# georgesterpu/avsr-tf1

Hardware: AMD Instinct MI355X
Metric: utterances/sec (train step) at B=64 T_a=500 T_v=75 (higher is better)
Workload: dtype f32; 1 GPU; c4: AV dual-attention (bimodal) video 1x256 + audio 3x256 uni-LSTM, scaled_luong, B=64 T_a=500x80 T_v=75 L=40; utterances_per_gpu=64, global_batch=64, T_a=500, F_a=80, T_v=75, F_v=128, T_dec=40, parallelism=dp1, video_frontend=resnet_cnn, launch=hipgraph, dropout=True

## Files before the change

### avsr-tf1_amd/csrc/gemm.hip

```cpp
#include "common.h"
#include "avsr_hip.h"
#include "prof.h"

namespace avsr {

constexpr int BM = 128, BN = 128, BK = 16;

struct MatView {
  const float* p;
  long ld;
  int T;
  long ldo;
  __device__ __forceinline__ const float* row(int r) const {
    return T ? p + (long)(r / T) * ldo + (long)(r % T) * ld : p + (long)r * ld;
  }
};

struct GemmArgs {
  MatView A, B;
  float* C; long ldc; int Tc; long ldoc;
  const float* bias;
  const float* alpha_dev;
  int M, N, K;
  int ta, tb;
  float alpha, beta;
  int splitk, kper;
  float* ws;
  long sA, sB, sC;
  int batch;
  float* cs_out; float cs_beta; float* cs_ws;
};

#define G_OOB ((int)0x80000000)
template <bool KC, bool VEC>
struct OperandLoader {
  __amdgpu_buffer_rsrc_t rs;
  int off[2];
  int q[2], r[2];
  bool ok;
  int ldb, ldob, T;
  int tail;
  int MN, mn;

  __device__ __forceinline__ void init(const MatView& S, int mn0, int k0, int MN_) {
    const int tid = threadIdx.x;
    rs = __builtin_amdgcn_make_buffer_rsrc(const_cast<float*>(S.p), 0, 0x80000000u, 0x00020000);
    ldb = (int)S.ld * 4; ldob = (int)S.ldo * 4; T = S.T; MN = MN_;
    if (KC) {
      mn = mn0 + (tid & 127);
      ok = mn < MN;
      const int ro = T ? (mn / T) * ldob + (mn % T) * ldb : mn * ldb;
#pragma unroll
      for (int p = 0; p < 2; ++p) off[p] = ro + (k0 + 4 * ((tid >> 7) + 2 * p)) * 4;
    } else {
      mn = mn0 + 4 * (tid & 31);
      ok = mn < MN;
#pragma unroll
      for (int p = 0; p < 2; ++p) {
        const int k = k0 + (tid >> 5) + 8 * p;
        q[p] = T ? k / T : 0; r[p] = T ? k % T : k;
        off[p] = mn * 4;
      }
    }
  }
  __device__ __forceinline__ void load(int k0, int kend, f32x4 (&out)[2]) {
    const int tid = threadIdx.x;
#pragma unroll
    for (int p = 0; p < 2; ++p) {
      int o, k;
      if (KC) { k = k0 + 4 * ((tid >> 7) + 2 * p); o = off[p]; off[p] += BK * 4; }
      else {
        k = k0 + (tid >> 5) + 8 * p;
        o = (T ? q[p] * ldob + r[p] * ldb : r[p] * ldb) + off[p];
        r[p] += BK;
        if (T) { while (r[p] >= T) { r[p] -= T; ++q[p]; } }
      }
      const bool in = ok && k < kend;
      typedef unsigned int u32x4_ __attribute__((ext_vector_type(4)));
      if (VEC) {
        out[p] = __builtin_bit_cast(f32x4, (u32x4_)__builtin_amdgcn_raw_buffer_load_b128(rs, in ? o : G_OOB, 0, 0));
      } else {
#pragma unroll
        for (int e = 0; e < 4; ++e) {
          const bool ine = in && (KC ? k + e < kend : mn + e < MN);
          out[p][e] = __builtin_bit_cast(float, (unsigned)__builtin_amdgcn_raw_buffer_load_b32(rs, ine ? o + 4 * e : G_OOB, 0, 0));
        }
      }
    }
  }
};

template <bool KC>
__device__ __forceinline__ void store_tile(float* T, const f32x4 (&r)[2]) {
  const int tid = threadIdx.x;
#pragma unroll
  for (int p = 0; p < 2; ++p) {
    if (KC) {
      const int mn = tid & 127;
      const int k = 4 * ((tid >> 7) + 2 * p);
#pragma unroll
      for (int e = 0; e < 4; ++e) T[(k + e) * BM + mn] = r[p][e];
    } else {
      const int k = (tid >> 5) + 8 * p;
      const int mn = 4 * (tid & 31);
      st4(&T[k * BM + mn], r[p]);
    }
  }
}

template <bool AKC, bool BKC, bool VECA, bool VECB>
__device__ __forceinline__ void gemm_body(const GemmArgs& g, const int bx, const int by, const int z) {
  __shared__ __attribute__((aligned(16))) float lds[2][2][BK * BM];
  const int tid = threadIdx.x, lane = tid & 63, wave = tid >> 6;
  const int wm = wave >> 1, wn = wave & 1;
  const int bz = z / g.splitk, sz = z % g.splitk;
  MatView A = g.A, B = g.B;
  A.p += (long)bz * g.sA;
  B.p += (long)bz * g.sB;
  const int m0 = by * BM, n0 = bx * BN;
  const int kbeg = sz * g.kper;
  const int kend = min(g.K, kbeg + g.kper);

  f32x16 acc[2][2];
#pragma unroll
  for (int i = 0; i < 2; ++i)
#pragma unroll
    for (int j = 0; j < 2; ++j)
#pragma unroll
      for (int r = 0; r < 16; ++r) acc[i][j][r] = 0.f;

  f32x4 ra[2][2], rb[2][2];
  OperandLoader<AKC, VECA> la;
  OperandLoader<BKC, VECB> lb;
  la.init(A, m0, kbeg, g.M);
  lb.init(B, n0, kbeg, g.N);
  la.load(kbeg, kend, ra[0]);
  lb.load(kbeg, kend, rb[0]);
  la.load(kbeg + BK, kend, ra[1]);
  lb.load(kbeg + BK, kend, rb[1]);
  const bool do_cs = !BKC && g.cs_out != nullptr && by == 0;
  f32x4 csum = {0.f, 0.f, 0.f, 0.f};
  store_tile<AKC>(lds[0][0], ra[0]);
  store_tile<BKC>(lds[0][1], rb[0]);
  if (do_cs) csum += rb[0][0] + rb[0][1];
  __syncthreads();

  auto ktile = [&](int k0, int buf, f32x4 (&ra_next)[2], f32x4 (&rb_next)[2], f32x4 (&ra_free)[2], f32x4 (&rb_free)[2]) {
    la.load(k0 + 2 * BK, kend, ra_free);
    lb.load(k0 + 2 * BK, kend, rb_free);
    const float* As = lds[buf][0];
    const float* Bs = lds[buf][1];
#pragma unroll
    for (int kk = 0; kk < BK / 2; ++kk) {
      const int k = 2 * kk + (lane >> 5);
      const float a0 = As[k * BM + wm * 64 + (lane & 31)];
      const float a1 = As[k * BM + wm * 64 + 32 + (lane & 31)];
      const float b0 = Bs[k * BN + wn * 64 + (lane & 31)];
      const float b1 = Bs[k * BN + wn * 64 + 32 + (lane & 31)];
      acc[0][0] = __builtin_amdgcn_mfma_f32_32x32x2f32(a0, b0, acc[0][0], 0, 0, 0);
      acc[0][1] = __builtin_amdgcn_mfma_f32_32x32x2f32(a0, b1, acc[0][1], 0, 0, 0);
      acc[1][0] = __builtin_amdgcn_mfma_f32_32x32x2f32(a1, b0, acc[1][0], 0, 0, 0);
      acc[1][1] = __builtin_amdgcn_mfma_f32_32x32x2f32(a1, b1, acc[1][1], 0, 0, 0);
    }
    store_tile<AKC>(lds[buf ^ 1][0], ra_next);
    store_tile<BKC>(lds[buf ^ 1][1], rb_next);
    if (do_cs) csum += rb_next[0] + rb_next[1];
    asm volatile("s_waitcnt lgkmcnt(0)\n\ts_barrier" ::: "memory");
  };
  for (int k0 = kbeg; k0 < kend; k0 += 2 * BK) {
    ktile(k0, 0, ra[1], rb[1], ra[0], rb[0]);
    if (k0 + BK < kend) ktile(k0 + BK, 1, ra[0], rb[0], ra[1], rb[1]);
  }

  if (!BKC && g.cs_out != nullptr) {
    float* red = &lds[0][0][0];
    if (do_cs) st4(red + (tid >> 5) * BN + 4 * (tid & 31), csum);
    __syncthreads();
    if (do_cs && tid < BN) {
      float v = 0.f;
#pragma unroll
      for (int r = 0; r < 8; ++r) v += red[r * BN + tid];
      const int col = n0 + tid;
      if (col < g.N) {
        if (g.splitk > 1) g.cs_ws[(long)z * g.N + col] = v;
        else g.cs_out[col] = g.cs_beta != 0.f ? v + g.cs_beta * g.cs_out[col] : v;
      }
    }
    __syncthreads();
  }
  const bool split = g.splitk > 1;
  const float alpha = g.alpha_dev ? g.alpha * g.alpha_dev[0] : g.alpha;
  const unsigned mTc = (g.Tc > 1 && g.M < 65536) ? (unsigned)(((1ull << 32) / (unsigned)g.Tc) + 1ull) : 0u;
  if (split) {
#pragma unroll
    for (int i = 0; i < 2; ++i)
#pragma unroll
      for (int j = 0; j < 2; ++j) {
        const int col = n0 + wn * 64 + j * 32 + (lane & 31);
        if (col >= g.N) continue;
        const int rbase = m0 + wm * 64 + i * 32 + 4 * (lane >> 5);
#pragma unroll
        for (int r = 0; r < 16; ++r) {
          const int row = rbase + (r & 3) + 8 * (r >> 2);
          if (row < g.M) g.ws[((long)z * g.M + row) * g.N + col] = acc[i][j][r];
        }
      }
    return;
  }
  const __amdgpu_buffer_rsrc_t c_rs = __builtin_amdgcn_make_buffer_rsrc(g.C + (long)bz * g.sC, 0, 0x80000000u, 0x00020000);
  int co[2][8];
  float old[2][8];
  auto prep = [&](int t, int (&cot)[8], float (&oldt)[8]) {
    const int i = t >> 2, j = (t >> 1) & 1, h = t & 1;
    const int col = n0 + wn * 64 + j * 32 + (lane & 31);
    const int rbase = m0 + wm * 64 + i * 32 + 4 * (lane >> 5);
#pragma unroll
    for (int rr = 0; rr < 8; ++rr) {
      const int r = h * 8 + rr;
      const int row = rbase + (r & 3) + 8 * (r >> 2);
      int o;
      if (!g.Tc) o = row * (int)g.ldc;
      else {
        const int qd = mTc ? (int)__umulhi((unsigned)row, mTc) : (g.Tc == 1 ? row : row / g.Tc);
        o = qd * (int)g.ldoc + (row - qd * g.Tc) * (int)g.ldc;
      }
      cot[rr] = (row < g.M && col < g.N) ? (o + col) * 4 : G_OOB;
    }
    if (g.beta != 0.f) {
#pragma unroll
      for (int rr = 0; rr < 8; ++rr) oldt[rr] = __builtin_bit_cast(float, (unsigned)__builtin_amdgcn_raw_buffer_load_b32(c_rs, cot[rr], 0, 0));
    }
  };
  prep(0, co[0], old[0]);
#pragma unroll
  for (int t = 0; t < 8; ++t) {
    if (t + 1 < 8) prep(t + 1, co[(t + 1) & 1], old[(t + 1) & 1]);
    const int i = t >> 2, j = (t >> 1) & 1, h = t & 1;
    const int col = n0 + wn * 64 + j * 32 + (lane & 31);
    const float bias_v = (g.bias && col < g.N) ? g.bias[col] : 0.f;
#pragma unroll
    for (int rr = 0; rr < 8; ++rr) {
      float v = alpha * acc[i][j][h * 8 + rr];
      if (g.beta != 0.f) v += g.beta * old[t & 1][rr];
      v += bias_v;
      __builtin_amdgcn_raw_buffer_store_b32(__builtin_bit_cast(unsigned, v), c_rs, co[t & 1][rr], 0, 0);
    }
  }
}

template <bool AKC, bool BKC, bool VECA, bool VECB>
__global__ __launch_bounds__(256, 3) void gemm_f32_kernel(GemmArgs g) {
  gemm_body<AKC, BKC, VECA, VECB>(g, blockIdx.x, blockIdx.y, blockIdx.z);
}

#define GEMM_GROUP_MAX 8
struct GemmGroup { int n; int blk_off[GEMM_GROUP_MAX + 1]; int gx[GEMM_GROUP_MAX], gy[GEMM_GROUP_MAX]; int red_off[GEMM_GROUP_MAX + 1]; GemmArgs g[GEMM_GROUP_MAX]; };

template <bool AKC, bool BKC, bool VECA, bool VECB>
__global__ __launch_bounds__(256, 3) void gemm_f32_group_kernel(const GemmGroup G) {
  int p = 0;
#pragma unroll
  for (int k = 1; k < GEMM_GROUP_MAX; ++k) if (k < G.n && (int)blockIdx.x >= G.blk_off[k]) p = k;
  p = __builtin_amdgcn_readfirstlane(p);
  const int b = blockIdx.x - G.blk_off[p];
  const int gx = G.gx[p], gy = G.gy[p];
  const int bx = b % gx, by = (b / gx) % gy, z = b / (gx * gy);
  gemm_body<AKC, BKC, VECA, VECB>(G.g[p], bx, by, z);
}

__device__ __forceinline__ void splitk_reduce_body(const GemmArgs& g, const long first, const long stride) {
  const long total = (long)g.batch * g.M * g.N;
  if (g.cs_out) {
    for (long col = first; col < g.N; col += stride) {
      float v = 0.f;
      int zz = 0;
      for (; zz + 8 <= g.splitk; zz += 8) {
        float w[8];
#pragma unroll
        for (int u = 0; u < 8; ++u) w[u] = g.cs_ws[(long)(zz + u) * g.N + col];
#pragma unroll
        for (int u = 0; u < 8; ++u) v += w[u];
      }
      for (; zz < g.splitk; ++zz) v += g.cs_ws[(long)zz * g.N + col];
      g.cs_out[col] = g.cs_beta != 0.f ? v + g.cs_beta * g.cs_out[col] : v;
    }
  }
  const bool vec = (g.N & 3) == 0 && ((uintptr_t)g.ws & 15) == 0 && ((uintptr_t)g.C & 15) == 0 && (g.ldc & 3) == 0 && (g.sC & 3) == 0 &&
                   (g.Tc == 0 || (g.ldoc & 3) == 0) && (!g.bias || ((uintptr_t)g.bias & 15) == 0);
  if (vec) {
    const long zs = (long)g.M * g.N;
    const float al = g.alpha_dev ? g.alpha * g.alpha_dev[0] : g.alpha;
    for (long i = first * 4; i < total; i += stride * 4) {
      const int col = (int)(i % g.N);
      const int row = (int)((i / g.N) % g.M);
      const int bz = (int)(i / zs);
      const float* w = g.ws + ((long)bz * g.splitk * g.M + row) * g.N + col;
      f32x4 s = {0.f, 0.f, 0.f, 0.f};
      int z = 0;
      for (; z + 8 <= g.splitk; z += 8) {
        f32x4 a[8];
#pragma unroll
        for (int u = 0; u < 8; ++u) a[u] = ld4(w + (z + u) * zs);
#pragma unroll
        for (int u = 0; u < 8; ++u) s += a[u];
      }
      for (; z < g.splitk; ++z) s += ld4(w + z * zs);
      float* c = g.C + (long)bz * g.sC +
                 (g.Tc ? (long)(row / g.Tc) * g.ldoc + (long)(row % g.Tc) * g.ldc : (long)row * g.ldc) + col;
      f32x4 v = al * s;
      if (g.beta != 0.f) v += g.beta * ld4(c);
      if (g.bias) v += ld4(g.bias + col);
      st4(c, v);
    }
    return;
  }
  for (long i = first; i < total; i += stride) {
    const int col = (int)(i % g.N);
    const int row = (int)((i / g.N) % g.M);
    const int bz = (int)(i / ((long)g.M * g.N));
    const float* w = g.ws + ((long)bz * g.splitk * g.M + row) * g.N + col;
    const long zs = (long)g.M * g.N;
    float s = 0.f;
    int z = 0;
    for (; z + 4 <= g.splitk; z += 4) {
      const float a0 = w[z * zs], a1 = w[(z + 1) * zs], a2 = w[(z + 2) * zs], a3 = w[(z + 3) * zs];
      s = (((s + a0) + a1) + a2) + a3;
    }
    for (; z < g.splitk; ++z) s += w[z * zs];
    float* c = g.C + (long)bz * g.sC +
               (g.Tc ? (long)(row / g.Tc) * g.ldoc + (long)(row % g.Tc) * g.ldc : (long)row * g.ldc) + col;
    float v = (g.alpha_dev ? g.alpha * g.alpha_dev[0] : g.alpha) * s;
    if (g.beta != 0.f) v += g.beta * *c;
    if (g.bias) v += g.bias[col];
    *c = v;
  }
}
__global__ void gemm_splitk_reduce_kernel(GemmArgs g) {
  splitk_reduce_body(g, (long)blockIdx.x * blockDim.x + threadIdx.x, (long)gridDim.x * blockDim.x);
}
__global__ void gemm_splitk_reduce_group_kernel(const GemmGroup G) {
  int p = 0;
#pragma unroll
  for (int k = 1; k < GEMM_GROUP_MAX; ++k) if (k < G.n && (int)blockIdx.x >= G.red_off[k]) p = k;
  p = __builtin_amdgcn_readfirstlane(p);
  if (G.g[p].splitk <= 1) return;
  const int nb = G.red_off[p + 1] - G.red_off[p];
  splitk_reduce_body(G.g[p], (long)(blockIdx.x - G.red_off[p]) * blockDim.x + threadIdx.x, (long)nb * blockDim.x);
}

static bool vec_ok(const avsr_mat* m, bool contig_is_k, int MN, int K) {
  const int contig = contig_is_k ? K : MN;
  return (((uintptr_t)m->ptr) % 16 == 0) && (m->ld % 4 == 0) && (contig % 4 == 0) && (m->T == 0 || m->ldo % 4 == 0);
}

}

static int gemm_prepare(const avsr_gemm_desc* d, avsr::GemmArgs& g, dim3* grid, int* cls) {
  using namespace avsr;
  if (!d || d->M <= 0 || d->N <= 0 || d->K < 0 || !d->A.ptr || !d->B.ptr || !d->C.ptr) return AVSR_ERR_ARG;
  g.A = MatView{d->A.ptr, d->A.ld, d->A.T, d->A.ldo};
  g.B = MatView{d->B.ptr, d->B.ld, d->B.T, d->B.ldo};
  g.C = d->C.ptr; g.ldc = d->C.ld; g.Tc = d->C.T; g.ldoc = d->C.ldo;
  g.bias = d->bias;
  g.alpha_dev = d->alpha_dev;
  g.M = d->M; g.N = d->N; g.K = d->K;
  g.ta = d->trans_a; g.tb = d->trans_b;
  g.alpha = d->alpha; g.beta = d->beta;
  g.batch = d->batch > 0 ? d->batch : 1;
  g.sA = d->stride_a; g.sB = d->stride_b; g.sC = d->stride_c;
  int splitk = d->splitk > 0 ? d->splitk : 1;
  if (splitk > 1 && (!d->workspace || d->workspace_floats < (long)g.batch * splitk * g.M * g.N)) return AVSR_ERR_ARG;
  int kper = ((g.K + splitk - 1) / splitk + BK - 1) / BK * BK;
  if (kper <= 0) kper = BK;
  splitk = (g.K + kper - 1) / kper;
  if (splitk < 1) splitk = 1;
  g.splitk = splitk; g.kper = kper; g.ws = d->workspace;
  g.cs_out = d->colsum; g.cs_beta = d->colsum_beta; g.cs_ws = nullptr;
  if (g.cs_out) {
    if (g.tb || g.batch != 1) return AVSR_ERR_UNSUPPORTED;
    if (splitk > 1) {
      if (d->workspace_floats < (long)splitk * g.M * g.N + (long)splitk * g.N) return AVSR_ERR_ARG;
      g.cs_ws = d->workspace + (long)splitk * g.M * g.N;
    }
  }
  const bool va = vec_ok(&d->A, g.ta == 0, g.M, g.K);
  const bool vb = vec_ok(&d->B, g.tb != 0, g.N, g.K);
  *grid = dim3((g.N + BN - 1) / BN, (g.M + BM - 1) / BM, g.batch * splitk);
  if ((long)d->A.ld * 4 >= (1L << 31) || (long)d->B.ld * 4 >= (1L << 31)) return AVSR_ERR_UNSUPPORTED;
  {
    const long rows = g.M - 1;
    const long last = (g.Tc ? (rows / g.Tc) * g.ldoc + (rows % g.Tc) * g.ldc : rows * g.ldc) + g.N;
    if (last * 4 >= (1L << 31)) return AVSR_ERR_UNSUPPORTED;
  }
  *cls = ((g.ta == 0) ? 8 : 0) | ((g.tb != 0) ? 4 : 0) | (va ? 2 : 0) | (vb ? 1 : 0);
  return AVSR_OK;
}

extern "C" int avsr_gemm_batch(const avsr_gemm_desc* descs, int32_t n, void* stream) {
  using namespace avsr;
  if (n <= 0) return AVSR_OK;
  if (!descs) return AVSR_ERR_ARG;
  hipStream_t s = (hipStream_t)stream;
  static thread_local GemmArgs ga[64];
  dim3 grids[64];
  int cls[64];
  if (n > 64) return AVSR_ERR_ARG;
  for (int i = 0; i < n; ++i) {
    const int rc = gemm_prepare(&descs[i], ga[i], &grids[i], &cls[i]);
    if (rc != AVSR_OK) return rc;
  }
  bool done[64] = {};
  for (int i = 0; i < n; ++i) {
    if (done[i]) continue;
    static thread_local GemmGroup G;
    G.n = 0;
    int blocks = 0, rblocks = 0;
    double flops = 0.0;
    bool any_split = false;
    for (int j = i; j < n && G.n < GEMM_GROUP_MAX; ++j) {
      if (done[j] || cls[j] != cls[i]) continue;
      const int p = G.n++;
      G.g[p] = ga[j];
      G.gx[p] = grids[j].x; G.gy[p] = grids[j].y;
      G.blk_off[p] = blocks; blocks += grids[j].x * grids[j].y * grids[j].z;
      G.red_off[p] = rblocks;
      if (ga[j].splitk > 1) {
        long tot = ((long)ga[j].batch * ga[j].M * ga[j].N + 255) / 256;
        rblocks += (int)(tot > 1024 ? 1024 : tot);
        any_split = true;
      } else rblocks += 1;
      flops += 2.0 * ga[j].M * ga[j].N * ga[j].K * ga[j].batch;
      done[j] = true;
    }
    G.blk_off[G.n] = blocks; G.red_off[G.n] = rblocks;
    ProfScope ps(PROF_GEMM, s, flops);
#define GG(AK, BK_, VA, VB) hipLaunchKernelGGL((gemm_f32_group_kernel<AK, BK_, VA, VB>), dim3(blocks), dim3(256), 0, s, G)
    switch (cls[i]) {
      case 15: GG(true, true, true, true); break;   case 14: GG(true, true, true, false); break;
      case 13: GG(true, true, false, true); break;  case 12: GG(true, true, false, false); break;
      case 11: GG(true, false, true, true); break;  case 10: GG(true, false, true, false); break;
      case 9: GG(true, false, false, true); break;  case 8: GG(true, false, false, false); break;
      case 7: GG(false, true, true, true); break;   case 6: GG(false, true, true, false); break;
      case 5: GG(false, true, false, true); break;  case 4: GG(false, true, false, false); break;
      case 3: GG(false, false, true, true); break;  case 2: GG(false, false, true, false); break;
      case 1: GG(false, false, false, true); break; default: GG(false, false, false, false); break;
    }
#undef GG
    AVSR_CHECK_LAUNCH();
    if (any_split) {
      hipLaunchKernelGGL(gemm_splitk_reduce_group_kernel, dim3(rblocks), dim3(256), 0, s, G);
      AVSR_CHECK_LAUNCH();
    }
  }
  return AVSR_OK;
}

extern "C" int avsr_gemm(const avsr_gemm_desc* d, void* stream) {
  using namespace avsr;
  GemmArgs g;
  dim3 grid;
  int cls = 0;
  const int rc = gemm_prepare(d, g, &grid, &cls);
  if (rc != AVSR_OK) return rc;
  hipStream_t s = (hipStream_t)stream;
  ProfScope ps(PROF_GEMM, s, 2.0 * g.M * g.N * g.K * g.batch);
#define GO(AK, BK_, VA, VB) hipLaunchKernelGGL((gemm_f32_kernel<AK, BK_, VA, VB>), grid, dim3(256), 0, s, g)
  switch (cls) {
    case 15: GO(true, true, true, true); break;   case 14: GO(true, true, true, false); break;
    case 13: GO(true, true, false, true); break;  case 12: GO(true, true, false, false); break;
    case 11: GO(true, false, true, true); break;  case 10: GO(true, false, true, false); break;
    case 9: GO(true, false, false, true); break;  case 8: GO(true, false, false, false); break;
    case 7: GO(false, true, true, true); break;   case 6: GO(false, true, true, false); break;
    case 5: GO(false, true, false, true); break;  case 4: GO(false, true, false, false); break;
    case 3: GO(false, false, true, true); break;  case 2: GO(false, false, true, false); break;
    case 1: GO(false, false, false, true); break; default: GO(false, false, false, false); break;
  }
#undef GO
  AVSR_CHECK_LAUNCH();
  if (g.splitk > 1) {
    const long total = (long)g.batch * g.M * g.N;
    int blocks = (int)((total + 255) / 256);
    if (blocks > 2048) blocks = 2048;
    hipLaunchKernelGGL(gemm_splitk_reduce_kernel, dim3(blocks), dim3(256), 0, s, g);
    AVSR_CHECK_LAUNCH();
  }
  return AVSR_OK;
}
```

Before: 5730 utterances/sec.

## Add per-shape GEMM planner with multiple MFMA tiles and skinny kernels

Adds a GEMM planner that picks a tile shape (128x128, 128x96, 96x128, 64x64) by padding waste and problem size, and routes N<=4 and K<=4 GEMMs to dedicated scalar skinny kernels. It also caps split-K for small problems. The aim is to cut padding waste and improve occupancy for the many small and odd-shaped GEMMs in the LSTM/attention step. In exchange, kernel dispatch grows more complex through runtime switches, and the 64x64 tile uses deeper register prefetch, which raises register pressure.

```diff
diff --git a/avsr-tf1_amd/csrc/gemm.hip b/avsr-tf1_amd/csrc/gemm.hip
--- a/avsr-tf1_amd/csrc/gemm.hip
+++ b/avsr-tf1_amd/csrc/gemm.hip
@@ -1,10 +1,17 @@
 #include "common.h"
 #include "avsr_hip.h"
 #include "prof.h"
+#include "gemm_plan.h"
 
 namespace avsr {
 
-constexpr int BM = 128, BN = 128, BK = 16;
+constexpr int BM = 128, BN = 128, BK = GEMM_BK;
+
+template <int TILE> struct TileCfg;
+template <> struct TileCfg<GEMM_TILE_128x128> { static constexpr int WM = 2, WN = 2, TI = 2, TJ = 2, PD = 2; };
+template <> struct TileCfg<GEMM_TILE_128x96>  { static constexpr int WM = 4, WN = 1, TI = 1, TJ = 3, PD = 2; };
+template <> struct TileCfg<GEMM_TILE_96x128>  { static constexpr int WM = 1, WN = 4, TI = 3, TJ = 1, PD = 2; };
+template <> struct TileCfg<GEMM_TILE_64x64>   { static constexpr int WM = 2, WN = 2, TI = 1, TJ = 1, PD = 4; };
 
 struct MatView {
   const float* p;
@@ -25,6 +32,7 @@
   int ta, tb;
   float alpha, beta;
   int splitk, kper;
+  int path, tile;
   float* ws;
   long sA, sB, sC;
   int batch;
@@ -108,36 +116,41 @@
   }
 }
 
-template <bool AKC, bool BKC, bool VECA, bool VECB>
-__device__ __forceinline__ void gemm_body(const GemmArgs& g, const int bx, const int by, const int z) {
-  __shared__ __attribute__((aligned(16))) float lds[2][2][BK * BM];
+template <int TILE, bool AKC, bool BKC, bool VECA, bool VECB>
+__device__ __forceinline__ void gemm_body(const GemmArgs& g, const int bx, const int by, const int z, float* lds_base) {
+  typedef TileCfg<TILE> TC;
+  constexpr int TI = TC::TI, TJ = TC::TJ, PD = TC::PD;
+  constexpr int BMt = TC::WM * TI * 32, BNt = TC::WN * TJ * 32;
+  float (*lds)[2][BK * BM] = reinterpret_cast<float (*)[2][BK * BM]>(lds_base);
   const int tid = threadIdx.x, lane = tid & 63, wave = tid >> 6;
-  const int wm = wave >> 1, wn = wave & 1;
+  const int wm = wave / TC::WN, wn = wave % TC::WN;
+  const int wr = wm * TI * 32, wc = wn * TJ * 32;
   const int bz = z / g.splitk, sz = z % g.splitk;
   MatView A = g.A, B = g.B;
   A.p += (long)bz * g.sA;
   B.p += (long)bz * g.sB;
-  const int m0 = by * BM, n0 = bx * BN;
+  const int m0 = by * BMt, n0 = bx * BNt;
   const int kbeg = sz * g.kper;
   const int kend = min(g.K, kbeg + g.kper);
 
-  f32x16 acc[2][2];
-#pragma unroll
-  for (int i = 0; i < 2; ++i)
-#pragma unroll
-    for (int j = 0; j < 2; ++j)
+  f32x16 acc[TI][TJ];
+#pragma unroll
+  for (int i = 0; i < TI; ++i)
+#pragma unroll
+    for (int j = 0; j < TJ; ++j)
 #pragma unroll
       for (int r = 0; r < 16; ++r) acc[i][j][r] = 0.f;
 
-  f32x4 ra[2][2], rb[2][2];
+  f32x4 ra[PD][2], rb[PD][2];
   OperandLoader<AKC, VECA> la;
   OperandLoader<BKC, VECB> lb;
-  la.init(A, m0, kbeg, g.M);
-  lb.init(B, n0, kbeg, g.N);
-  la.load(kbeg, kend, ra[0]);
-  lb.load(kbeg, kend, rb[0]);
-  la.load(kbeg + BK, kend, ra[1]);
-  lb.load(kbeg + BK, kend, rb[1]);
+  la.init(A, m0, kbeg, min(g.M, m0 + BMt));
+  lb.init(B, n0, kbeg, min(g.N, n0 + BNt));
+#pragma unroll
+  for (int u = 0; u < PD; ++u) {
+    la.load(kbeg + u * BK, kend, ra[u]);
+    lb.load(kbeg + u * BK, kend, rb[u]);
+  }
   const bool do_cs = !BKC && g.cs_out != nullptr && by == 0;
   f32x4 csum = {0.f, 0.f, 0.f, 0.f};
   store_tile<AKC>(lds[0][0], ra[0]);
@@ -146,37 +159,39 @@
   __syncthreads();
 
   auto ktile = [&](int k0, int buf, f32x4 (&ra_next)[2], f32x4 (&rb_next)[2], f32x4 (&ra_free)[2], f32x4 (&rb_free)[2]) {
-    la.load(k0 + 2 * BK, kend, ra_free);
-    lb.load(k0 + 2 * BK, kend, rb_free);
+    la.load(k0 + PD * BK, kend, ra_free);
+    lb.load(k0 + PD * BK, kend, rb_free);
     const float* As = lds[buf][0];
     const float* Bs = lds[buf][1];
 #pragma unroll
     for (int kk = 0; kk < BK / 2; ++kk) {
       const int k = 2 * kk + (lane >> 5);
-      const float a0 = As[k * BM + wm * 64 + (lane & 31)];
-      const float a1 = As[k * BM + wm * 64 + 32 + (lane & 31)];
-      const float b0 = Bs[k * BN + wn * 64 + (lane & 31)];
-      const float b1 = Bs[k * BN + wn * 64 + 32 + (lane & 31)];
-      acc[0][0] = __builtin_amdgcn_mfma_f32_32x32x2f32(a0, b0, acc[0][0], 0, 0, 0);
-      acc[0][1] = __builtin_amdgcn_mfma_f32_32x32x2f32(a0, b1, acc[0][1], 0, 0, 0);
-      acc[1][0] = __builtin_amdgcn_mfma_f32_32x32x2f32(a1, b0, acc[1][0], 0, 0, 0);
-      acc[1][1] = __builtin_amdgcn_mfma_f32_32x32x2f32(a1, b1, acc[1][1], 0, 0, 0);
+      float a[TI], b[TJ];
+#pragma unroll
+      for (int i = 0; i < TI; ++i) a[i] = As[k * BM + wr + i * 32 + (lane & 31)];
+#pragma unroll
+      for (int j = 0; j < TJ; ++j) b[j] = Bs[k * BN + wc + j * 32 + (lane & 31)];
+#pragma unroll
+      for (int i = 0; i < TI; ++i)
+#pragma unroll
+        for (int j = 0; j < TJ; ++j) acc[i][j] = __builtin_amdgcn_mfma_f32_32x32x2f32(a[i], b[j], acc[i][j], 0, 0, 0);
     }
     store_tile<AKC>(lds[buf ^ 1][0], ra_next);
     store_tile<BKC>(lds[buf ^ 1][1], rb_next);
     if (do_cs) csum += rb_next[0] + rb_next[1];
     asm volatile("s_waitcnt lgkmcnt(0)\n\ts_barrier" ::: "memory");
   };
-  for (int k0 = kbeg; k0 < kend; k0 += 2 * BK) {
-    ktile(k0, 0, ra[1], rb[1], ra[0], rb[0]);
-    if (k0 + BK < kend) ktile(k0 + BK, 1, ra[0], rb[0], ra[1], rb[1]);
+  for (int k0 = kbeg; k0 < kend; k0 += PD * BK) {
+#pragma unroll
+    for (int u = 0; u < PD; ++u)
+      if (u == 0 || k0 + u * BK < kend) ktile(k0 + u * BK, u & 1, ra[(u + 1) % PD], rb[(u + 1) % PD], ra[u], rb[u]);
   }
 
   if (!BKC && g.cs_out != nullptr) {
     float* red = &lds[0][0][0];
     if (do_cs) st4(red + (tid >> 5) * BN + 4 * (tid & 31), csum);
     __syncthreads();
-    if (do_cs && tid < BN) {
+    if (do_cs && tid < BNt) {
       float v = 0.f;
 #pragma unroll
       for (int r = 0; r < 8; ++r) v += red[r * BN + tid];
@@ -193,12 +208,12 @@
   const unsigned mTc = (g.Tc > 1 && g.M < 65536) ? (unsigned)(((1ull << 32) / (unsigned)g.Tc) + 1ull) : 0u;
   if (split) {
 #pragma unroll
-    for (int i = 0; i < 2; ++i)
-#pragma unroll
-      for (int j = 0; j < 2; ++j) {
-        const int col = n0 + wn * 64 + j * 32 + (lane & 31);
+    for (int i = 0; i < TI; ++i)
+#pragma unroll
+      for (int j = 0; j < TJ; ++j) {
+        const int col = n0 + wc + j * 32 + (lane & 31);
         if (col >= g.N) continue;
-        const int rbase = m0 + wm * 64 + i * 32 + 4 * (lane >> 5);
+        const int rbase = m0 + wr + i * 32 + 4 * (lane >> 5);
 #pragma unroll
         for (int r = 0; r < 16; ++r) {
           const int row = rbase + (r & 3) + 8 * (r >> 2);
@@ -211,9 +226,9 @@
   int co[2][8];
   float old[2][8];
   auto prep = [&](int t, int (&cot)[8], float (&oldt)[8]) {
-    const int i = t >> 2, j = (t >> 1) & 1, h = t & 1;
-    const int col = n0 + wn * 64 + j * 32 + (lane & 31);
-    const int rbase = m0 + wm * 64 + i * 32 + 4 * (lane >> 5);
+    const int i = (t >> 1) / TJ, j = (t >> 1) % TJ, h = t & 1;
+    const int col = n0 + wc + j * 32 + (lane & 31);
+    const int rbase = m0 + wr + i * 32 + 4 * (lane >> 5);
 #pragma unroll
     for (int rr = 0; rr < 8; ++rr) {
       const int r = h * 8 + rr;
@@ -233,10 +248,10 @@
   };
   prep(0, co[0], old[0]);
 #pragma unroll
-  for (int t = 0; t < 8; ++t) {
-    if (t + 1 < 8) prep(t + 1, co[(t + 1) & 1], old[(t + 1) & 1]);
-    const int i = t >> 2, j = (t >> 1) & 1, h = t & 1;
-    const int col = n0 + wn * 64 + j * 32 + (lane & 31);
+  for (int t = 0; t < 2 * TI * TJ; ++t) {
+    if (t + 1 < 2 * TI * TJ) prep(t + 1, co[(t + 1) & 1], old[(t + 1) & 1]);
+    const int i = (t >> 1) / TJ, j = (t >> 1) % TJ, h = t & 1;
+    const int col = n0 + wc + j * 32 + (lane & 31);
     const float bias_v = (g.bias && col < g.N) ? g.bias[col] : 0.f;
 #pragma unroll
     for (int rr = 0; rr < 8; ++rr) {
@@ -248,9 +263,92 @@
   }
 }
 
+__device__ __forceinline__ float* c_row(const GemmArgs& g, int bz, int row) {
+  return g.C + (long)bz * g.sC + (g.Tc ? (long)(row / g.Tc) * g.ldoc + (long)(row % g.Tc) * g.ldc : (long)row * g.ldc);
+}
+__device__ __forceinline__ void skinny_store(const GemmArgs& g, int bz, int row, int col, float s) {
+  float* c = c_row(g, bz, row) + col;
+  float v = (g.alpha_dev ? g.alpha * g.alpha_dev[0] : g.alpha) * s;
+  if (g.beta != 0.f) v += g.beta * *c;
+  if (g.bias) v += g.bias[col];
+  *c = v;
+}
+
+__device__ __forceinline__ void gemm_skinny_n_body(const GemmArgs& g, const int bx, const int z, float* lds) {
+  const int tid = threadIdx.x;
+  const int rl = g.ta ? (tid & 15) : (tid >> 4);
+  const int kl = g.ta ? (tid >> 4) : (tid & 15);
+  const int bz = z / g.splitk, sz = z % g.splitk;
+  MatView A = g.A, B = g.B;
+  A.p += (long)bz * g.sA;
+  B.p += (long)bz * g.sB;
+  const int row = bx * 16 + rl;
+  const int kbeg = sz * g.kper;
+  const int kend = min(g.K, kbeg + g.kper);
+  float acc[4] = {0.f, 0.f, 0.f, 0.f};
+  if (row < g.M) {
+    const float* arow = g.ta ? A.p + row : A.row(row);
+#pragma unroll 4
+    for (int k = kbeg + kl; k < kend; k += 16) {
+      const float a = g.ta ? A.row(k)[row] : arow[k];
+#pragma unroll
+      for (int n = 0; n < 4; ++n)
+        if (n < g.N) acc[n] += a * (g.tb ? B.row(n)[k] : B.row(k)[n]);
+    }
+  }
+  st4(lds + (kl * 16 + rl) * 4, f32x4{acc[0], acc[1], acc[2], acc[3]});
+  __syncthreads();
+  if (tid < 64) {
+    const int r = tid >> 2, n = tid & 3;
+    float v = 0.f;
+#pragma unroll
+    for (int q = 0; q < 16; ++q) v += lds[(q * 16 + r) * 4 + n];
+    const int orow = bx * 16 + r;
+    if (orow < g.M && n < g.N) {
+      if (g.splitk > 1) g.ws[((long)z * g.M + orow) * g.N + n] = v;
+      else skinny_store(g, bz, orow, n, v);
+    }
+  }
+}
+
+__device__ __forceinline__ void gemm_skinny_k_body(const GemmArgs& g, const int bx, const int z) {
+  const unsigned nq = ((unsigned)g.N + 3u) / 4u;
+  const unsigned idx = (unsigned)bx * 256u + threadIdx.x;
+  if (idx >= (unsigned)g.M * nq) return;
+  const int row = (int)(idx / nq), c0 = 4 * (int)(idx % nq);
+  MatView A = g.A, B = g.B;
+  A.p += (long)z * g.sA;
+  B.p += (long)z * g.sB;
+  float s[4] = {0.f, 0.f, 0.f, 0.f};
+#pragma unroll
+  for (int k = 0; k < 4; ++k) {
+    if (k >= g.K) break;
+    const float a = g.ta ? A.row(k)[row] : A.row(row)[k];
+#pragma unroll
+    for (int e = 0; e < 4; ++e)
+      if (c0 + e < g.N) s[e] += a * (g.tb ? B.row(c0 + e)[k] : B.row(k)[c0 + e]);
+  }
+#pragma unroll
+  for (int e = 0; e < 4; ++e)
+    if (c0 + e < g.N) skinny_store(g, z, row, c0 + e, s[e]);
+}
+
+template <bool AKC, bool BKC, bool VECA, bool VECB>
+__device__ __forceinline__ void gemm_dispatch(const GemmArgs& g, const int bx, const int by, const int z, float* lds) {
+  if (g.path == GEMM_PATH_SKINNY_N) { gemm_skinny_n_body(g, bx, z, lds); return; }
+  if (g.path == GEMM_PATH_SKINNY_K) { gemm_skinny_k_body(g, bx, z); return; }
+  switch (g.tile) {
+    case GEMM_TILE_128x96: gemm_body<GEMM_TILE_128x96, AKC, BKC, VECA, VECB>(g, bx, by, z, lds); break;
+    case GEMM_TILE_96x128: gemm_body<GEMM_TILE_96x128, AKC, BKC, VECA, VECB>(g, bx, by, z, lds); break;
+    case GEMM_TILE_64x64:  gemm_body<GEMM_TILE_64x64, AKC, BKC, VECA, VECB>(g, bx, by, z, lds); break;
+    default:               gemm_body<GEMM_TILE_128x128, AKC, BKC, VECA, VECB>(g, bx, by, z, lds); break;
+  }
+}
+
 template <bool AKC, bool BKC, bool VECA, bool VECB>
 __global__ __launch_bounds__(256, 3) void gemm_f32_kernel(GemmArgs g) {
-  gemm_body<AKC, BKC, VECA, VECB>(g, blockIdx.x, blockIdx.y, blockIdx.z);
+  __shared__ __attribute__((aligned(16))) float lds[2 * 2 * BK * BM];
+  gemm_dispatch<AKC, BKC, VECA, VECB>(g, blockIdx.x, blockIdx.y, blockIdx.z, lds);
 }
 
 #define GEMM_GROUP_MAX 8
@@ -265,7 +363,8 @@
   const int b = blockIdx.x - G.blk_off[p];
   const int gx = G.gx[p], gy = G.gy[p];
   const int bx = b % gx, by = (b / gx) % gy, z = b / (gx * gy);
-  gemm_body<AKC, BKC, VECA, VECB>(G.g[p], bx, by, z);
+  __shared__ __attribute__((aligned(16))) float lds[2 * 2 * BK * BM];
+  gemm_dispatch<AKC, BKC, VECA, VECB>(G.g[p], bx, by, z, lds);
 }
 
 __device__ __forceinline__ void splitk_reduce_body(const GemmArgs& g, const long first, const long stride) {
@@ -368,13 +467,12 @@
   g.alpha = d->alpha; g.beta = d->beta;
   g.batch = d->batch > 0 ? d->batch : 1;
   g.sA = d->stride_a; g.sB = d->stride_b; g.sC = d->stride_c;
-  int splitk = d->splitk > 0 ? d->splitk : 1;
-  if (splitk > 1 && (!d->workspace || d->workspace_floats < (long)g.batch * splitk * g.M * g.N)) return AVSR_ERR_ARG;
-  int kper = ((g.K + splitk - 1) / splitk + BK - 1) / BK * BK;
-  if (kper <= 0) kper = BK;
-  splitk = (g.K + kper - 1) / kper;
-  if (splitk < 1) splitk = 1;
-  g.splitk = splitk; g.kper = kper; g.ws = d->workspace;
+  const int hint = d->splitk > 0 ? d->splitk : 1;
+  if (hint > 1 && (!d->workspace || d->workspace_floats < (long)g.batch * hint * g.M * g.N)) return AVSR_ERR_ARG;
+  const GemmPlan plan = gemm_plan(g.M, g.N, g.K, g.batch, hint, d->colsum != nullptr);
+  const int splitk = plan.splitk;
+  g.splitk = splitk; g.kper = plan.kper; g.ws = d->workspace;
+  g.path = plan.path; g.tile = plan.tile;
   g.cs_out = d->colsum; g.cs_beta = d->colsum_beta; g.cs_ws = nullptr;
   if (g.cs_out) {
     if (g.tb || g.batch != 1) return AVSR_ERR_UNSUPPORTED;
@@ -385,7 +483,7 @@
   }
   const bool va = vec_ok(&d->A, g.ta == 0, g.M, g.K);
   const bool vb = vec_ok(&d->B, g.tb != 0, g.N, g.K);
-  *grid = dim3((g.N + BN - 1) / BN, (g.M + BM - 1) / BM, g.batch * splitk);
+  *grid = dim3(plan.gx, plan.gy, g.batch * splitk);
   if ((long)d->A.ld * 4 >= (1L << 31) || (long)d->B.ld * 4 >= (1L << 31)) return AVSR_ERR_UNSUPPORTED;
   {
     const long rows = g.M - 1;
diff --git a/avsr-tf1_amd/csrc/gemm_plan.h b/avsr-tf1_amd/csrc/gemm_plan.h
--- /dev/null
+++ b/avsr-tf1_amd/csrc/gemm_plan.h
@@ -0,0 +1,79 @@
+#pragma once
+
+namespace avsr {
+
+constexpr int GEMM_BK = 16;
+
+enum GemmPath {
+  GEMM_PATH_MFMA = 0,
+  GEMM_PATH_SKINNY_N = 1,
+  GEMM_PATH_SKINNY_K = 2,
+};
+
+enum GemmTile { GEMM_TILE_128x128 = 0, GEMM_TILE_128x96 = 1, GEMM_TILE_96x128 = 2, GEMM_TILE_64x64 = 3, GEMM_TILES = 4 };
+
+struct GemmPlan {
+  int path, tile;
+  int bm, bn;
+  int gx, gy;
+  int splitk, kper;
+};
+
+inline int gemm_tile_bm(int t) { return t == GEMM_TILE_96x128 ? 96 : t == GEMM_TILE_64x64 ? 64 : 128; }
+inline int gemm_tile_bn(int t) { return t == GEMM_TILE_128x96 ? 96 : t == GEMM_TILE_64x64 ? 64 : 128; }
+
+inline long gemm_padded(int M, int N, int bm, int bn) {
+  return (long)((M + bm - 1) / bm) * bm * (long)((N + bn - 1) / bn) * bn;
+}
+
+inline GemmPlan gemm_plan(int M, int N, int K, int batch, int splitk_hint, bool colsum) {
+  GemmPlan p;
+  int splitk = splitk_hint > 0 ? splitk_hint : 1;
+  int kper = ((K + splitk - 1) / splitk + GEMM_BK - 1) / GEMM_BK * GEMM_BK;
+  if (kper <= 0) kper = GEMM_BK;
+  splitk = (K + kper - 1) / kper;
+  if (splitk < 1) splitk = 1;
+  p.splitk = splitk; p.kper = kper;
+  if (batch < 1) batch = 1;
+
+  if (!colsum && K <= 4 && (long)M * N < (1L << 31)) {
+    p.path = GEMM_PATH_SKINNY_K; p.tile = 0; p.bm = 1; p.bn = 1024;
+    p.gx = (int)(((long)M * ((N + 3) / 4) + 255) / 256); p.gy = 1;
+    p.splitk = 1; p.kper = GEMM_BK;
+    return p;
+  }
+  if (!colsum && N <= 4) {
+    p.path = GEMM_PATH_SKINNY_N; p.tile = 0; p.bm = 16; p.bn = 4;
+    p.gx = (M + 15) / 16; p.gy = 1;
+    return p;
+  }
+
+  const long tiles128 = (long)((M + 127) / 128) * ((N + 127) / 128) * batch;
+  const bool small = (double)M * N * K * batch <= 750e6 && tiles128 < 128 && K <= 1024;
+  int tile = GEMM_TILE_128x128;
+  if (M <= 64 || N <= 64 || small) tile = GEMM_TILE_64x64;
+  else {
+    const long p128 = gemm_padded(M, N, 128, 128), p96n = gemm_padded(M, N, 128, 96), p96m = gemm_padded(M, N, 96, 128);
+    long best = p128;
+    if (p96n * 10 <= p128 * 9 && p96n < best) { best = p96n; tile = GEMM_TILE_128x96; }
+    if (p96m * 10 <= p128 * 9 && p96m < best) { best = p96m; tile = GEMM_TILE_96x128; }
+  }
+  if ((M + gemm_tile_bm(tile) - 1) / gemm_tile_bm(tile) > 65535) tile = GEMM_TILE_128x128;
+  p.path = GEMM_PATH_MFMA; p.tile = tile;
+  p.bm = gemm_tile_bm(tile); p.bn = gemm_tile_bn(tile);
+  p.gx = (N + p.bn - 1) / p.bn; p.gy = (M + p.bm - 1) / p.bm;
+
+  if (small && tile == GEMM_TILE_64x64 && p.splitk > 1) {
+    const long tiles = (long)p.gx * p.gy * batch;
+    long cap = tiles >= 256 ? 1 : (512 + tiles - 1) / tiles;
+    if (cap > K / 128) cap = K / 128;
+    if (cap < 1) cap = 1;
+    if (cap < p.splitk) {
+      p.kper = (int)(((K + cap - 1) / cap + GEMM_BK - 1) / GEMM_BK * GEMM_BK);
+      p.splitk = (K + p.kper - 1) / p.kper;
+    }
+  }
+  return p;
+}
+
+}
```

Result: no change. 5770 utterances/sec (median of 6 runs) (+0.7%).
